# muellan/metacache

Hardware: AMD Instinct MI355X
Metric: Mreads/min (150 bp) (higher is better)
Workload: dtype u32

## Files before the change

### metacache_amd/csrc/gw_kernels.hip

```cpp
#include "device_common.h"

#include <algorithm>
#include <cstdlib>

namespace mcamd {

namespace {

constexpr uint32_t kGwNone = 0xFFFFFFFFu;
constexpr uint32_t kGwRounds = 128;
constexpr uint32_t kGwLoads = kGwRounds / 16;

struct __attribute__((packed, aligned(4))) U4 { uint32_t x, y, z, w; };

__device__ __forceinline__ uint32_t gw_block_shift(uint32_t maxWin)
{
    const uint32_t D = maxWin > 1 ? maxWin - 1 : 1;
    const uint32_t A = 32u - (uint32_t)__builtin_clz(64u * D - 1u);
    return A < 8u ? 8u : A;
}

template <uint32_t T1LOG2, uint32_t T2LOG2>
struct GwBloom {
    static constexpr uint32_t kW1 = (1u << T1LOG2) / 32, kW2 = (1u << T2LOG2) / 32, kWords = kW1 + kW2;
// ... 60 lines not shown
    }
    __device__ __forceinline__ static bool seen(const uint32_t* bits, uint32_t key)
    {
        const uint32_t h = hash(key), m = mask_of(h);
        return (bits[seen_index(h)] & m) == m;
    }
};

struct GwFrame {
    uint32_t A, D, blockMask, inner;
    uint32_t shv, Dsh, twoDsh;
    __device__ __forceinline__ explicit GwFrame(uint32_t maxWin, bool fine = false)
    {
        A = gw_block_shift(maxWin); D = maxWin > 1 ? maxWin - 1 : 0u;
        if (fine) { A = 32u - (uint32_t)__builtin_clz((D > 1u ? D : 2u) - 1u); A = A < 8u ? 8u : A; }
        blockMask = (1u << A) - 1u; inner = (1u << A) - 2u * D;
        const uint32_t sh = 32u - A;
        asm volatile("v_mov_b32 %0, %1" : "=v"(shv) : "s"(sh));
        Dsh = D << sh; twoDsh = (2u * D) << sh;
    }
    __device__ __forceinline__ bool edge(uint32_t v) const
    {
        uint32_t t;
        asm("v_lshl_add_u32 %0, %1, %2, %3" : "=v"(t) : "v"(v), "v"(shv), "s"(Dsh));
        return t < twoDsh;
    }
};

__device__ __forceinline__ void gw_fill_rounds(uint64_t* T, uint32_t lane, uint32_t r0, uint32_t Rc, uint32_t start, uint32_t myR, uint32_t sz, uint64_t pay)
{
    for (uint32_t i = lane; i < kGwRounds; i += 64) if (r0 + i >= Rc) T[i] = 0ull;
    const uint32_t jlo = r0 > start ? r0 - start : 0u, jhi = min(myR, r0 + kGwRounds > start ? r0 + kGwRounds - start : 0u);
    for (uint32_t j = jlo; j < jhi; ++j) T[start + j - r0] = (pay + 16ull * j) | ((uint64_t)min(16u, sz - 16u * j) << 40);
}
__device__ __forceinline__ uint32_t gw_lane_value(uint32_t v, int src) { return (uint32_t)__builtin_amdgcn_ds_bpermute(src << 2, (int)v); }
__device__ __forceinline__ void gw_fill_rounds_scan(uint64_t* T, uint32_t* E, uint32_t lane, uint32_t Rc, uint32_t start, uint32_t myR, uint32_t sz, uint64_t pay)
{
    E[lane] = 0u; E[lane + 64u] = 0u;
    wave_lds_sync();
    if (myR && start < kGwRounds) E[start] = lane + 1u;
    wave_lds_sync();
    uint32_t lo = wave_incl_scan_max_u32(E[lane]);
    uint32_t hi = max(wave_incl_scan_max_u32(E[lane + 64u]), rdlane(lo, 63));
    const uint32_t payLo = (uint32_t)pay, payHi = (uint32_t)(pay >> 32);
#pragma unroll
    for (uint32_t h = 0; h < 2; ++h) {
        const uint32_t slot = lane + 64u * h, who = h ? hi : lo;
        const int src = (int)(who ? who - 1u : 0u);
        const uint32_t eStart = gw_lane_value(start, src), eSz = gw_lane_value(sz, src);
        const uint32_t eLo = gw_lane_value(payLo, src), eHi = gw_lane_value(payHi, src);
        const uint32_t j = slot - eStart;
        const uint64_t ep = ((uint64_t)eHi << 32) | eLo;
        T[slot] = (who && slot < Rc) ? ((ep + 16ull * j) | ((uint64_t)min(16u, eSz - 16u * j) << 40)) : 0ull;
    }
}
__device__ __forceinline__ void gw_fill_rounds_scan_at(uint64_t* T, uint32_t* E, uint32_t lane, uint32_t r0, uint32_t Rc, uint32_t start, uint32_t myR, uint32_t sz, uint64_t pay)
{
    E[lane] = 0u; E[lane + 64u] = 0u;
    wave_lds_sync();
    if (myR && start < r0 + kGwRounds && start + myR > r0) E[start > r0 ? start - r0 : 0u] = lane + 1u;
    wave_lds_sync();
    uint32_t lo = wave_incl_scan_max_u32(E[lane]);
    uint32_t hi = max(wave_incl_scan_max_u32(E[lane + 64u]), rdlane(lo, 63));
    const uint32_t payLo = (uint32_t)pay, payHi = (uint32_t)(pay >> 32);
#pragma unroll
    for (uint32_t h = 0; h < 2; ++h) {
        const uint32_t slot = lane + 64u * h, who = h ? hi : lo;
        const int src = (int)(who ? who - 1u : 0u);
        const uint32_t eStart = gw_lane_value(start, src), eSz = gw_lane_value(sz, src);
        const uint32_t eLo = gw_lane_value(payLo, src), eHi = gw_lane_value(payHi, src);
        const uint32_t j = r0 + slot - eStart;
        const uint64_t ep = ((uint64_t)eHi << 32) | eLo;
        T[slot] = (who && r0 + slot < Rc) ? ((ep + 16ull * j) | ((uint64_t)min(16u, eSz - 16u * j) << 40)) : 0ull;
    }
}
__device__ __forceinline__ uint4 gw_left_as_is()
{
    uint4 r;
    asm volatile("" : "=v"(r.x), "=v"(r.y), "=v"(r.z), "=v"(r.w));
    return r;
}
template <bool BARE = false>
__device__ __forceinline__ void gw_load_rounds(const uint64_t* T, const uint32_t* __restrict__ values32, uint32_t grp, uint32_t sub4, uint4 (&x)[kGwLoads],
                                               uint32_t nl = kGwLoads)
{
#pragma unroll
    for (uint32_t u = 0; u < kGwLoads; ++u) {
        x[u] = make_uint4(kGwNone, kGwNone, kGwNone, kGwNone);
        if (u >= nl) continue;
        if constexpr (BARE) { x[u] = gw_left_as_is(); x[u].x = kGwNone; }
        const uint64_t rd = T[u * 16 + grp];
        if (sub4 < (uint32_t)(rd >> 40)) {
            const U4 t = *reinterpret_cast<const U4*>(values32 + (rd & 0xFFFFFFFFFFull) + sub4);
            x[u] = make_uint4(t.x, t.y, t.z, t.w);
        }
    }
}
template <class Bloom, bool LEAVE = false>
__device__ __forceinline__ void gw_mark_rounds(uint32_t* bits, const uint4 (&x)[kGwLoads], uint32_t A, uint32_t nl = kGwLoads)
{
#pragma unroll
    for (uint32_t u = 0; u < kGwLoads; ++u) {
        if (u >= nl) { if constexpr (LEAVE) break; else continue; }
        if (x[u].x != kGwNone) Bloom::mark4(bits, x[u].x >> A, x[u].y >> A, x[u].z >> A, x[u].w >> A);
    }
}
struct GwSink { uint32_t* dst; uint32_t room, n2; uint32_t* shared = nullptr; };
__device__ __forceinline__ uint32_t gw_reserve(uint32_t* shared, uint32_t tot)
{
    uint32_t at = 0;
    if (tot && __builtin_amdgcn_mbcnt_hi(~0u, __builtin_amdgcn_mbcnt_lo(~0u, 0u)) == 0u) at = atomicAdd(shared, tot);
    return (uint32_t)__builtin_amdgcn_readfirstlane((int)at);
}
template <class Bloom, bool FINE = false>
__device__ __forceinline__ void gw_take(const uint32_t* bits, const GwFrame& F, GwSink& S, uint32_t v, bool valid)
{
    const uint32_t key = v >> F.A;
    const bool keep = valid & (FINE ? (Bloom::twice(bits, key) | Bloom::seen(bits, key - 1u) | Bloom::seen(bits, key + 1u)) : (Bloom::twice(bits, key) | F.edge(v)));
    const uint64_t m = __ballot(keep);
    if (S.shared) S.n2 = gw_reserve(S.shared, (uint32_t)__popcll(m));
    if (keep) {
        const uint32_t at = __builtin_amdgcn_mbcnt_hi((uint32_t)(m >> 32), __builtin_amdgcn_mbcnt_lo((uint32_t)m, S.n2));
        if (at < S.room) S.dst[at] = v;
    }
    S.n2 += (uint32_t)__popcll(m);
}
constexpr int kGwFits = 0, kGwLaneRoom = 1, kGwWaveRoom = 2;
template <class Bloom, int CHECK, bool FINE = false>
__device__ __forceinline__ void gw_take4(const uint32_t* bits, const GwFrame& F, GwSink& S, const uint4 x, const int32_t rem)
{
    const uint32_t v[4] = {x.x, x.y, x.z, x.w};
    uint32_t m[4], wd[4];
    uint32_t mlo[FINE ? 4 : 1], wlo[FINE ? 4 : 1], mhi[FINE ? 4 : 1], whi[FINE ? 4 : 1];
#pragma unroll
    for (int j = 0; j < 4; ++j) {
        const uint32_t key = v[j] >> F.A;
        const uint32_t h = Bloom::hash(key);
        m[j] = h;
        wd[j] = bits[Bloom::twice_index(Bloom::seen_index(h), h)];
        if constexpr (FINE) {
            const uint32_t h0 = Bloom::hash(key - 1u), h1 = Bloom::hash(key + 1u);
            mlo[j] = Bloom::mask_of(h0); wlo[j] = bits[Bloom::seen_index(h0)];
            mhi[j] = Bloom::mask_of(h1); whi[j] = bits[Bloom::seen_index(h1)];
        }
    }
    uint64_t km[4]; bool kb[4];
#pragma unroll
    for (int j = 0; j < 4; ++j) {
        const bool valid = rem > j, hit = Bloom::twice_hit_h(wd[j], m[j]);
        if constexpr (FINE) {
            const bool lo = (wlo[j] & mlo[j]) == mlo[j], hi = (whi[j] & mhi[j]) == mhi[j];
            kb[j] = valid & (hit | lo | hi);
            km[j] = __ballot(valid) & (__ballot(hit) | __ballot(lo) | __ballot(hi));
        } else {
            const bool edge = F.edge(v[j]);
            kb[j] = valid & (hit | edge);
            km[j] = __ballot(valid) & (__ballot(hit) | __ballot(edge));
        }
    }
    if (S.shared) S.n2 = gw_reserve(S.shared, (uint32_t)(__popcll(km[0]) + __popcll(km[1]) + __popcll(km[2]) + __popcll(km[3])));
    uint32_t n2 = S.n2;
    if constexpr (CHECK == kGwWaveRoom) {
        const uint32_t end = n2 + (uint32_t)__popcll(km[0]) + (uint32_t)__popcll(km[1]) + (uint32_t)__popcll(km[2]) + (uint32_t)__popcll(km[3]);
        if (end <= S.room) {
#pragma unroll
            for (int j = 0; j < 4; ++j) {
                if (kb[j]) {
                    const uint32_t mine = __builtin_amdgcn_mbcnt_hi((uint32_t)(km[j] >> 32), __builtin_amdgcn_mbcnt_lo((uint32_t)km[j], 0u));
                    (S.dst + n2)[mine] = v[j];
                }
                n2 += (uint32_t)__popcll(km[j]);
            }
        }
        S.n2 = end;
        return;
    }
#pragma unroll
    for (int j = 0; j < 4; ++j) {
        if (kb[j]) {
// ... 471 lines not shown
        const uint32_t mv = wave_min_u32(hh == mh ? hv : kGwNone);
        const uint32_t winner = __ffsll((unsigned long long)__ballot(hh == mh && hv == mv)) - 1;
        const uint32_t d = rdlane(hd, winner);
        if constexpr (TAX) {
            const uint32_t g = rdlane(hg, winner);
#pragma unroll
            for (uint32_t r = 0; r < PER; ++r) if (ptax[r] == g) live &= ~(1u << r);
        } else {
            const uint32_t from = mv - tab.gwGap, span = 2u * tab.gwGap;
#pragma unroll
            for (uint32_t r = 0; r < PER; ++r) if (v[r] - from <= span) live &= ~(1u << r);
        }
        if (lane == rnd) { wv = mv; wh = mh; wd = d; }
        strong += mh >= 2 ? 1u : 0u;
    }
    owv = wv; owh = wh; owd = wd;
    return strong;
}

template <bool TAX>
__device__ __forceinline__ bool gw_winners_out(const uint32_t lane, const uint32_t K, const uint32_t wv, const uint32_t wh, const uint32_t wd,
                                               const uint32_t wt, const uint32_t wlo, const uint32_t whi, mc_candidate_dev* __restrict__ out,
                                               uint32_t (&pickLo)[kLaneK], uint32_t (&pickHi)[kLaneK])
{
    bool again = false;
    if constexpr (!TAX) {
#pragma unroll
        for (uint32_t i = 0; i + 1 < kLaneK; ++i) {
            const uint32_t ti = rdlane(wt, i);
            again = again || (__ballot(lane > i && lane < K && wt == ti && ti != 0xFFFFFFFFu) != 0);
        }
    }
#pragma unroll
    for (uint32_t i = 0; i < kLaneK; ++i) { pickLo[i] = rdlane(wlo, i); pickHi[i] = rdlane(whi, i); }
    if (lane < K) {
        mc_candidate_dev e; e.tgt = wt; e.hits = wh; e.end = wv - wlo; e.beg = e.end - wd;
        if (wv == kGwNone) { e.tgt = 0xFFFFFFFFu; e.hits = 0; e.beg = 0; e.end = 0; }
        out[lane] = e;
    }
    return again;
}

}

namespace {

__device__ __forceinline__ void lk_store_entries(const Workspace& ws, const uint32_t fbase, const uint32_t nf, const uint32_t lane, const uint32_t sz, const uint64_t pay,
                                                 const uint64_t fm, const uint64_t sm, const uint32_t lincl)
{
    const uint32_t nent = (uint32_t)__popcll(fm), n1 = (uint32_t)__popcll(sm), lsz = sz > 1u ? sz : 0u;
    const uint32_t below = __builtin_amdgcn_mbcnt_hi((uint32_t)(fm >> 32), __builtin_amdgcn_mbcnt_lo((uint32_t)fm, 0u));
    const uint32_t sbelow = __builtin_amdgcn_mbcnt_hi((uint32_t)(sm >> 32), __builtin_amdgcn_mbcnt_lo((uint32_t)sm, 0u));
    if (sz != 0u) {
        const uint32_t slot = sz == 1u ? sbelow : n1 + (below - sbelow);
        const uint32_t off = sz == 1u ? slot : n1 + lincl - lsz;
        ws.psize[fbase + slot] = sz | ((off & kEntOffMask) << 16);
        ws.ppay[fbase + slot] = pay;
    } else if (lane < nf) ws.psize[fbase + nent + (lane - below)] = 0u;
}
__device__ __forceinline__ void lk_store_entries(const Workspace& ws, const uint32_t fbase, const uint32_t nf, const uint32_t lane, const uint32_t sz, const uint64_t pay)
{
    lk_store_entries(ws, fbase, nf, lane, sz, pay, __ballot(sz != 0u), __ballot(sz == 1u), wave_incl_scan_u32(sz > 1u ? sz : 0u, lane));
}
__device__ __forceinline__ void lk_load_entries(const Workspace& ws, const DeviceTable& tab, const uint32_t s, const uint32_t q, const uint32_t lane,
                                                uint32_t& fbase, uint32_t& nf, uint32_t& sz, uint64_t& pay)
{
    const uint32_t o0 = ws.winOff[q];
    fbase = o0 * s; nf = (ws.winOff[q + 1] - o0) * s;
    const uint32_t f = lane < nf ? ws.features[fbase + lane] : 0xFFFFFFFFu;
    const uint64_t e = f != 0xFFFFFFFFu ? tab.direct[f] : 0ull;
    sz = (uint32_t)e & 0xFFFFu; pay = direct_payload(e);
}

struct GwEntRecord {
    const uint4* rec;
    __device__ __forceinline__ uint2 where() const { const uint4 r6 = *rec; return make_uint2(r6.y, rec_entries(r6.z)); }
    __device__ __forceinline__ void load(const Workspace& ws, const DeviceTable&, uint32_t, uint32_t fbase, uint32_t nent, uint32_t lane, uint32_t& sz, uint64_t& pay) const
    {
        sz = lane < nent ? (ws.psize[fbase + lane] & 0xFFFFu) : 0u;
        pay = lane < nent ? ws.ppay[fbase + lane] : 0ull;
    }
    __device__ __forceinline__ void leave(const Workspace&, const DeviceTable&, uint32_t, uint32_t) const {}
};
struct GwEntLookup {
    uint32_t fbase, nent, s;
    __device__ __forceinline__ uint2 where() const { return make_uint2(fbase, nent); }
    __device__ __forceinline__ void load(const Workspace& ws, const DeviceTable& tab, uint32_t q, uint32_t, uint32_t, uint32_t lane, uint32_t& sz, uint64_t& pay) const
    {
        uint32_t fb, nf;
        lk_load_entries(ws, tab, s, q, lane, fb, nf, sz, pay);
    }
    __device__ __forceinline__ void leave(const Workspace& ws, const DeviceTable& tab, uint32_t q, uint32_t lane) const
    {
        uint32_t fb, nf, sz; uint64_t pay;
        lk_load_entries(ws, tab, s, q, lane, fb, nf, sz, pay);
        lk_store_entries(ws, fb, nf, lane, sz, pay);
    }
};

struct GwPend {
    bool pend = false;
    uint32_t q = 0, wv = kGwNone, whd = 0, dir = 0, b0 = 0, b1 = 0, b2 = 0;
    __device__ __forceinline__ void bases(const DeviceTable& tab)
    {
        b0 = b1 = b2 = 0u;
        if (pend && wv != kGwNone) { b0 = tab.gwBase[dir]; b1 = tab.gwBase[dir + 1]; b2 = tab.gwBase[min(dir + 2, tab.gwTargets)]; }
    }
    template <bool TAX, class Ent>
    __device__ __forceinline__ void finish(const uint32_t lane, const uint32_t K, const DeviceTable& tab, const Workspace& ws, mc_candidate_dev* __restrict__ cands, const Ent& ent)
    {
        if (!pend) return;
        uint32_t t = 0xFFFFFFFFu, lo = 0, hi = 0;
        if (wv != kGwNone) {
            t = dir; lo = b0; hi = b1;
            if (wv >= b1) { ++t; lo = b1; hi = b2; }
            while (wv >= hi) { ++t; lo = hi; hi = tab.gwBase[t + 1]; }
        }
        uint32_t plo[kLaneK], phi[kLaneK];
        const bool again = gw_winners_out<TAX>(lane, K, wv, whd & 0xFFFFu, whd >> 16, t, lo, hi, cands + (size_t)q * K, plo, phi);
        if (again) ent.leave(ws, tab, q, lane);
        if (lane == 0) {
            if (again) { ws.hitScan[q] = ws.qstat[q].hits; ws.qflag[q] = kFlagCands; }
            else ws.qflag[q] = kFlagDone;
        }
        pend = false;
    }
};

template <uint32_t LOG2S, bool TAX, bool DEFER, bool LONG = false, class GetV, class Ent>
__device__ __forceinline__ bool gw_count_read(const uint32_t q, const Ent& ent, const uint32_t n2, const uint32_t maxWin, GetV&& getv,
                                              uint2* slots, uint32_t* ck, uint64_t* T, const uint32_t lane, const uint32_t grp, const uint32_t sub4,
                                              const uint32_t K, const uint32_t* __restrict__ taxkey, const DeviceTable& tab, const Workspace& ws,
                                              mc_candidate_dev* __restrict__ cands, GwPend& P)
{
    constexpr uint32_t kSlots = 1u << LOG2S, kList = kSlots / 2;
    {
        uint4* k4 = reinterpret_cast<uint4*>(slots);
#pragma unroll
        for (uint32_t i = 0; i < kSlots * 8 / 16 / 64; ++i) k4[i * 64 + lane] = make_uint4(kGwNone, 0u, kGwNone, 0u);
    }
    wave_lds_sync();
    uint32_t pickLo[kLaneK], pickHi[kLaneK];
#pragma unroll
    for (uint32_t i = 0; i < kLaneK; ++i) { pickLo[i] = 0; pickHi[i] = 0; }
    uint32_t strong = 0, wv = kGwNone, wh = 0, wd = 0;
    bool again = false;
    mc_candidate_dev* out = cands + (size_t)q * K;
    if constexpr (DEFER) P.bases(tab);
    uint32_t C = 0;
    auto body = [&](auto perc) {
        constexpr uint32_t PER = decltype(perc)::value;
        uint32_t v[PER];
#pragma unroll
        for (uint32_t r = 0; r < PER; ++r) v[r] = getv(r);
        C = gw_count_numbers<LOG2S, PER, LONG ? kList : 0xFFFFFFFFu>(v, slots, ck, lane);
    };
    const uint32_t per = (n2 + 63u) / 64u;
    if constexpr (LOG2S == 9) {
        if (per <= 1) body(std::integral_constant<uint32_t, 1>{});
        else if (per <= 2) body(std::integral_constant<uint32_t, 2>{});
        else if (per <= 3) body(std::integral_constant<uint32_t, 3>{});
        else if (!LONG || per <= 4) body(std::integral_constant<uint32_t, 4>{});
        else if constexpr (LONG) {
            if (per <= 6) body(std::integral_constant<uint32_t, 6>{});
            else body(std::integral_constant<uint32_t, 8>{});
        }
    } else if constexpr (LOG2S == 10) {
        if (per <= 6) body(std::integral_constant<uint32_t, 6>{});
        else body(std::integral_constant<uint32_t, 8>{});
    } else {
        if (per <= 10) body(std::integral_constant<uint32_t, 10>{});
        else if (per <= 12) body(std::integral_constant<uint32_t, 12>{});
        else body(std::integral_constant<uint32_t, kList / 64>{});
    }
    C = __builtin_amdgcn_readfirstlane(C);
    wave_lds_sync();
    if constexpr (LONG) {
        if (C > kList) {
            if constexpr (DEFER) P.template finish<TAX>(lane, K, tab, ws, cands, ent);
// ... 106 lines not shown
                ent.leave(ws, tab, q, lane);
                if (lane == 0) { ws.hitScan[q] = ws.qstat[q].hits; ws.qflag[q] = kFlagCands; }
                done = false;
            }
        }
    }
    if (done && lane == 0) ws.qflag[q] = kFlagDone;
    wave_lds_sync();
    return true;
}

}

#ifndef MC_GW_COUNT_WPE
#define MC_GW_COUNT_WPE 6
#endif
template <uint32_t LOG2S, uint32_t WAVES, bool TAX>
__global__ __launch_bounds__(WAVES * 64, LOG2S == 9 ? MC_GW_COUNT_WPE : LOG2S == 10 ? 5 : 1) void gw_count_kernel(BatchView b, uint32_t s, DeviceTable tab, Workspace ws, uint32_t K,
                                                                                             const uint32_t* __restrict__ taxkey, mc_candidate_dev* __restrict__ cands,
                                                                                             uint32_t minN2)
{
    constexpr uint32_t kSlots = 1u << LOG2S, kList = kSlots / 2;
    static_assert(kGwRounds * 8 <= kSlots * 8, "step D's round table lives in the slot table, which is done with by then");
    __shared__ __attribute__((aligned(16))) uint2 slotS[WAVES][kSlots];
    __shared__ uint32_t ckS[WAVES][kList];
    const uint32_t lane = threadIdx.x & 63u, wave = __builtin_amdgcn_readfirstlane(threadIdx.x >> 6);
    uint2* slots = slotS[wave];
    uint32_t* ck = ckS[wave];
    uint64_t* T = reinterpret_cast<uint64_t*>(slotS[wave]);
    const uint32_t total = ws.midCount[kCntFilter];
    const uint4* __restrict__ work = ws.midList + list_at(kListFiltered, b.n);
    const uint4* __restrict__ work6 = ws.midList + list_at(kListFilter, b.n);
    const uint32_t nWaves = gridDim.x * WAVES;
    const uint32_t w0 = blockIdx.x * WAVES + wave;
    const uint32_t grp = lane >> 2, sub4 = (lane & 3u) * 4u;
    const uint32_t* __restrict__ pool = reinterpret_cast<const uint32_t*>(ws.bigPool);
    constexpr uint32_t kPre = LOG2S <= 10 ? kList / 64 : 1;
    uint32_t pre[kPre];
    auto fetch = [&](uint32_t off, uint32_t n) {
        if constexpr (LOG2S <= 10) {
#pragma unroll
            for (uint32_t r = 0; r < kPre; ++r) pre[r] = r * 64 + lane < n ? pool[off + r * 64 + lane] : kGwNone;
        }
    };
    constexpr bool kDefer = LOG2S <= 10;
    GwPend P;
    const uint32_t nmine = LOG2S == 9 ? total : ws.midCount[LOG2S == 10 ? kCnt512 : kCnt1024];
    const uint32_t kStep = LOG2S == 9 ? 64u : min(8u, max(1u, (nmine + nWaves - 1) / nWaves));
    const uint32_t* __restrict__ side = ws.sideList + list_at(LOG2S == 10 ? kSide512 : kSide1024, b.n);
    for (uint32_t chunk = w0 * kStep; chunk < nmine; chunk += nWaves * kStep) {
      const bool inb = lane < kStep && chunk + lane < nmine;
      const uint32_t myW = LOG2S == 9 ? chunk + lane : (inb ? side[chunk + lane] : 0u);
      const uint4 myRec = inb ? work[myW] : make_uint4(0, 0, kGwFallback, 0);
      uint64_t todo = __ballot(myRec.z <= kList && (minN2 == 0 || myRec.z > minN2) && myRec.w <= kHashWin);
      if (todo) { const uint32_t j = (uint32_t)__ffsll((unsigned long long)todo) - 1; fetch(rdlane(myRec.y, j), rdlane(myRec.z, j)); }
      while (todo) {
        const uint32_t j = (uint32_t)__ffsll((unsigned long long)todo) - 1;
        todo &= todo - 1;
        const uint32_t w = rdlane(myW, j), q = rdlane(myRec.x, j), n2 = rdlane(myRec.z, j), maxWin = rdlane(myRec.w, j);
        const uint32_t* __restrict__ src = pool + rdlane(myRec.y, j);
        uint32_t cur[kPre];
#pragma unroll
        for (uint32_t r = 0; r < kPre; ++r) cur[r] = pre[r];
        if (todo) { const uint32_t jn = (uint32_t)__ffsll((unsigned long long)todo) - 1; fetch(rdlane(myRec.y, jn), rdlane(myRec.z, jn)); }
        gw_count_read<LOG2S, TAX, kDefer>(q, GwEntRecord{work6 + w}, n2, maxWin, [&](uint32_t r) -> uint32_t {
            if constexpr (LOG2S <= 10) return cur[r < kPre ? r : 0];
            else return r * 64 + lane < n2 ? src[r * 64 + lane] : kGwNone;
        }, slots, ck, T, lane, grp, sub4, K, taxkey, tab, ws, cands, P);
      }
    }
    if constexpr (kDefer) { P.bases(tab); P.template finish<TAX>(lane, K, tab, ws, cands, GwEntRecord{work6}); }
}

constexpr uint32_t kGwCounted = 0x80000000u;

template <uint32_t WAVES, uint32_t TLOG2, bool TAX, uint32_t WPE = MC_GW_FILTER_WPE, bool LOOKUP = false>
__global__ __launch_bounds__(WAVES * 64, WPE) void gw_filter_count_kernel(BatchView b, DeviceTable tab, Workspace ws, uint32_t K, const uint32_t* __restrict__ taxkey,
                                                                                 mc_candidate_dev* __restrict__ cands, const uint32_t s)
{
    using Bloom = GwBloom<TLOG2, TLOG2>;
    constexpr uint32_t kKeep = WPE >= 6 ? 384 : 512;
    static_assert(kGwRounds * 8 >= 256 * 4, "the distinct numbers' slots take the place of the round table");
    constexpr bool kSeven = WPE >= 7;
    __shared__ __attribute__((aligned(16))) uint32_t bitS[WAVES][Bloom::kWords];
    __shared__ __attribute__((aligned(16))) uint64_t roundS[kSeven ? 1 : WAVES][kSeven ? 1 : kGwRounds];
    __shared__ __attribute__((aligned(16))) uint32_t keptS[WAVES][kKeep];
    uint32_t lane = threadIdx.x & 63u;
    const uint32_t wave = __builtin_amdgcn_readfirstlane(threadIdx.x >> 6);
    uint32_t* bits = bitS[wave];
    uint64_t* T = kSeven ? reinterpret_cast<uint64_t*>(bits) : roundS[kSeven ? 0 : wave];
    uint32_t* kept = keptS[wave];
    const uint32_t total = LOOKUP ? b.n : ws.midCount[kCntFilter];
    uint4* const work = ws.midList + list_at(kListFilter, b.n);
    uint4* __restrict__ outRec = ws.midList + list_at(kListFiltered, b.n);
    const uint32_t nWaves = gridDim.x * WAVES;
    const uint32_t w0 = blockIdx.x * WAVES + wave;
    auto load_rec = [&](uint32_t w) -> uint4 { return (!LOOKUP && w < total) ? work[w] : make_uint4(0, 0, 0, 0); };
    const uint64_t sliceCap = ws.bigPoolCap / nWaves;
    uint32_t* const slice = reinterpret_cast<uint32_t*>(ws.bigPool) + (uint64_t)w0 * sliceCap;
    uint64_t sliceUsed = (LOOKUP && ws.sliceFill) ? ws.sliceFill[w0] : 0u;
    uint32_t deferred = 0;
    uint4 rec = load_rec(w0), recNext = load_rec(w0 + nWaves);
    uint32_t esz = 0; uint64_t epay = 0;
    auto load_entries = [&](const uint4& r) {
        if constexpr (LOOKUP) return;
        const uint32_t ne = rec_hits(r.z) <= kGwSmallH ? min(rec_entries(r.z), 64u) : 0u;
        esz = lane < ne ? ws.psize[r.y + lane] : 0u;
        epay = lane < ne ? ws.ppay[r.y + lane] : 0ull;
    };
    load_entries(rec);
    constexpr uint32_t kLkSkip = 0xFFFFFFFFu;
    auto load_raw = [&](uint32_t q) -> uint32_t {
        uint32_t raw = 0u;
        if (LOOKUP && q < b.n && lane < 3u) raw = *(lane < 2u ? ws.winOff + q + lane : ws.qflag + q);
        return raw;
    };
    auto decode_raw = [&](uint32_t raw) -> uint2 {
        const uint32_t o0 = rdlane(raw, 0), nf = (rdlane(raw, 1) - o0) * s;
        return (LOOKUP && rdlane(raw, 2) == kFlagProbe && nf <= 64u) ? make_uint2(o0 * s, nf) : make_uint2(kLkSkip, 0u);
    };
    auto load_feat = [&](const uint2& m) -> uint32_t { return (m.x != kLkSkip && lane < m.y) ? ws.features[m.x + lane] : 0xFFFFFFFFu; };
    uint2 mA = make_uint2(kLkSkip, 0u), mB = mA;
    uint32_t lkFeat = 0xFFFFFFFFu, lkNfeat = 0, lkRaw = 0; uint64_t lkEnt = 0;
    if constexpr (LOOKUP) {
        mA = decode_raw(load_raw(w0)); mB = decode_raw(load_raw(w0 + nWaves));
        const uint32_t f0 = load_feat(mA);
        lkFeat = load_feat(mB);
        lkRaw = load_raw(w0 + 2 * nWaves);
        lkNfeat = (uint32_t)__popcll(__ballot(f0 != 0xFFFFFFFFu));
        lkEnt = f0 != 0xFFFFFFFFu ? tab.direct[f0] : 0ull;
    }
    uint32_t grp = lane >> 2, sub4 = (lane & 3u) * 4u;
    auto hide_lane = [&]() {
        if constexpr (LOOKUP) { asm volatile("" : "+v"(lane)); grp = lane >> 2; sub4 = (lane & 3u) * 4u; }
    };
    GwPend P;
    for (uint32_t w = w0; w < total; w += nWaves) {
      bool advanced = false;
      auto advance = [&]() {
          if constexpr (LOOKUP) { lkFeat = load_feat(mB); lkRaw = load_raw(w + 3 * nWaves); advanced = true; }
      };
      do {
        uint32_t q, nent, H, maxWin, sz, fbase = 0, nfs = 0; uint64_t pay;
        uint32_t rix = 0xFFFFFFFFu;
        if constexpr (!LOOKUP) {
            q = rec.x; nent = rec_entries(rec.z); H = rec_hits(rec.z); maxWin = rec.w;
            sz = esz & 0xFFFFu; pay = epay;
            rec = recNext;
            recNext = load_rec(w + 2 * nWaves);
            load_entries(rec);
        } else {
            hide_lane();
            const uint2 cur = mA; const uint64_t e = lkEnt; const uint32_t nfeat = lkNfeat;
            const uint2 mC = decode_raw(lkRaw);
            lkNfeat = (uint32_t)__popcll(__ballot(lkFeat != 0xFFFFFFFFu));
            lkEnt = lkFeat != 0xFFFFFFFFu ? tab.direct[lkFeat] : 0ull;
            mA = mB; mB = mC;
            if (cur.x == kLkSkip) continue;
            q = w; fbase = cur.x; nfs = cur.y;
            sz = (uint32_t)e & 0xFFFFu; pay = direct_payload(e);
            const uint64_t fm = __ballot(sz != 0u), sm = __ballot(sz == 1u);
            nent = (uint32_t)__popcll(fm);
            const uint32_t n1 = (uint32_t)__popcll(sm), lsz = sz > 1u ? sz : 0u;
            const uint32_t lincl = wave_incl_scan_u32(lsz, lane);
            H = n1 + rdlane(lincl, 63);
            maxWin = b.max_win(q);
            if (lane == 0) { QueryStat qs; qs.hits = H; qs.nfeat = nfeat; qs.nfound = nent; qs.nsteps = nfeat; ws.qstat[q] = qs; }
            if (H == 0) {
                if (lane < K) { mc_candidate_dev ev; ev.tgt = 0xFFFFFFFFu; ev.hits = 0; ev.beg = 0; ev.end = 0; cands[(size_t)q * K + lane] = ev; }
                if (lane == 0) { ws.hitScan[q] = 0u; ws.qflag[q] = kFlagDone; }
                continue;
            }
            const uint32_t cls = read_class(H, nent, maxWin, ClassLimits{ws.bigMin, tab.gwGap, true});
            if (lane == 0) {
                ws.hitScan[q] = segment_hits(H, cls);
                ws.qflag[q] = cls != kClassWave ? kFlagMid : kFlagCands;
                if (cls != kClassWave && cls != kClassFilter) {
                    const uint32_t at = atomicAdd(&ws.midCount[class_counter(cls)], 1u);
                    ws.midList[list_at(class_list(cls), b.n) + at] = as_uint4(work_record(q, fbase, nent, H, maxWin));
                }
            }
            if (cls != kClassFilter) { lk_store_entries(ws, fbase, nfs, lane, sz, pay, fm, sm, lincl); continue; }
        }
        auto entries_out = [&]() { if constexpr (LOOKUP) GwEntLookup{fbase, nent, s}.leave(ws, tab, q, lane); };
        auto slot_of = [&]() -> uint32_t {
            if constexpr (!LOOKUP) return w;
            else {
                if (rix == 0xFFFFFFFFu) {
                    uint32_t at = 0;
                    if (lane == 0) { at = atomicAdd(&ws.midCount[kCntFilter], 1u); work[at] = as_uint4(work_record(q, fbase, nent, H, maxWin)); }
                    rix = rdlane(at, 0);
                }
                return rix;
            }
        };
        const uint32_t myR = sz > 1 ? (sz + 15u) >> 4 : 0u;
        const uint32_t incl = wave_incl_scan_u32(myR, lane), Rc = rdlane(incl, 63);
        if (H > kGwSmallH || nent > 64u || Rc > kGwRounds || maxWin > tab.gwGap || sliceCap - sliceUsed < kGwRounds * 16u + 64u) {
            if constexpr (LOOKUP) lk_store_entries(ws, fbase, nfs, lane, sz, pay);
            const uint32_t at = slot_of();
            if (lane == 0) outRec[at] = make_uint4(q, 0u, kGwDefer, maxWin);
            ++deferred;
            continue;
        }
        auto clear_bits = [&]() {
            uint4* z4 = reinterpret_cast<uint4*>(bits);
#pragma unroll
            for (uint32_t i = 0; i < Bloom::kWords / 4 / 64; ++i) z4[i * 64 + lane] = make_uint4(0, 0, 0, 0);
        };
        if constexpr (!kSeven) clear_bits();
        gw_fill_rounds_scan(T, kept, lane, Rc, incl - myR, myR, sz, pay);
        wave_lds_sync();
        const GwFrame F(maxWin);
        const uint32_t nl = (Rc + 15u) >> 4;
        const uint32_t svLow = sz == 1 ? (uint32_t)pay : 0u;
        const uint32_t svBase = sz == 1 ? tab.gwBase[(uint32_t)(pay >> 32)] : kGwNone;
        uint4 x[kGwLoads];
        gw_load_rounds<LOOKUP>(T, tab.values32, grp, sub4, x, nl);
        uint32_t svTop = svBase;
        uint32_t rems = 0;
        if constexpr (kSeven) {
            rems = gw_pack_rems<LOOKUP>(T, grp, sub4, nl);
            hide_lane();
            wave_lds_sync();
            clear_bits();
            wave_lds_sync();
            if constexpr (LOOKUP) asm volatile("" : "+v"(svTop));
        }
        const uint32_t sv = svTop + svLow;
        auto take_rounds = [&](auto check, GwSink& S) {
            constexpr int CHECK = decltype(check)::value;
            if constexpr (kSeven) gw_take_rounds_packed<Bloom, CHECK, LOOKUP>(bits, rems, F, S, x, nl);
            else gw_take_rounds<Bloom, CHECK>(bits, T, F, S, grp, sub4, x, nl);
        };
        if (sv != kGwNone) Bloom::mark(bits, sv >> F.A);
        gw_mark_rounds<Bloom, LOOKUP>(bits, x, F.A, nl);
        hide_lane();
        wave_lds_sync();
        const bool here = maxWin <= kHashWin;
        uint32_t n2;
        if (here) {
            GwSink S{kept, kKeep, 0u};
            gw_take<Bloom>(bits, F, S, sv, sv != kGwNone);
            take_rounds(std::integral_constant<int, LOOKUP ? kGwWaveRoom : kGwLaneRoom>{}, S);
            n2 = S.n2;
        } else {
            GwSink S{slice + sliceUsed, (uint32_t)min((uint64_t)kGwMaxKept, sliceCap - sliceUsed), 0u};
            gw_take<Bloom>(bits, F, S, sv, sv != kGwNone);
            take_rounds(std::integral_constant<int, kGwFits>{}, S);
            n2 = S.n2;
        }
        if (here && n2 <= kKeep) {
            hide_lane();
            advance();
            if constexpr (!LOOKUP) { if (lane == 0) outRec[w] = make_uint4(q, 0u, kGwCounted | n2, maxWin); }
            wave_lds_sync();
            auto count = [&](const auto& ent) {
                return gw_count_read<9, TAX, true, true>(q, ent, n2, maxWin,
                                        [&](uint32_t r) -> uint32_t { return r * 64 + lane < n2 ? kept[r * 64 + lane] : kGwNone; },
                                        reinterpret_cast<uint2*>(bits), kSeven ? kept : reinterpret_cast<uint32_t*>(T), kSeven ? reinterpret_cast<uint64_t*>(kept) : T,
                                        lane, grp, sub4, K, taxkey, tab, ws, cands, P);
            };
            bool counted;
            if constexpr (LOOKUP) counted = count(GwEntLookup{fbase, nent, s});
            else counted = count(GwEntRecord{work + w});
            if (!counted && kSeven) {
                entries_out();
                const uint32_t at = slot_of();
                if (lane == 0) outRec[at] = make_uint4(q, 0u, kGwDefer, maxWin);
                ++deferred;
                wave_lds_sync();
            } else if (!counted) {
#pragma unroll
                for (uint32_t r = 0; r < kKeep / 64; ++r) if (r * 64 + lane < n2) slice[sliceUsed + r * 64 + lane] = kept[r * 64 + lane];
                entries_out();
                const uint32_t at = slot_of();
                if (lane == 0) outRec[at] = make_uint4(q, (uint32_t)((uint64_t)w0 * sliceCap + sliceUsed), n2, maxWin);
                sliceUsed += n2;
                wave_lds_sync();
            }
            continue;
        }
        if (here) {
            GwSink S{slice + sliceUsed, (uint32_t)min((uint64_t)kGwMaxKept, sliceCap - sliceUsed), 0u};
            gw_take<Bloom>(bits, F, S, sv, sv != kGwNone);
            take_rounds(std::integral_constant<int, kGwFits>{}, S);
            n2 = S.n2;
        }
        const uint32_t room = (uint32_t)min((uint64_t)kGwMaxKept, sliceCap - sliceUsed);
        const bool fallback = n2 > room;
        entries_out();
        const uint32_t at = slot_of();
        if (lane == 0) {
            if (fallback) { ws.hitScan[q] = H; ws.qflag[q] = kFlagCands; outRec[at] = make_uint4(q, 0u, kGwFallback, maxWin); }
            else outRec[at] = make_uint4(q, (uint32_t)((uint64_t)w0 * sliceCap + sliceUsed), n2, maxWin);
        }
        if (!fallback) sliceUsed += n2;
        wave_lds_sync();
      } while (false);
      if (!advanced) advance();
    }
    P.bases(tab);
    if constexpr (LOOKUP) P.template finish<TAX>(lane, K, tab, ws, cands, GwEntLookup{0u, 0u, s});
    else P.template finish<TAX>(lane, K, tab, ws, cands, GwEntRecord{work});
    if (lane == 0) {
        if (ws.sliceFill) ws.sliceFill[w0] = (uint32_t)sliceUsed;
        if (deferred) atomicAdd(&ws.midCount[kCntSecond], deferred);
    }
}

constexpr uint32_t kGwBigSorted = 8192;

template <bool TAX>
__device__ __forceinline__ void gw_sorted_scan(const uint32_t* __restrict__ g, const uint32_t first, const uint32_t end, const uint32_t D,
                                               const DeviceTable& tab, const uint32_t* __restrict__ taxkey, const uint32_t K, uint32_t* ring,
                                               const uint32_t lane, LaneCand (&top)[kLaneK], uint32_t (&toptax)[kLaneK])
{
    uint32_t cT = 0xFFFFFFFFu, cHits = 0, cBeg = 0, cEnd = 0, cLo = 0, cHi = 0;
    uint32_t lowFst = 0;
    uint32_t gnext = first + lane < end ? g[first + lane] : 0xFFFFFFFFu;
    uint32_t dnext = gnext != 0xFFFFFFFFu ? tab.gwDir[gnext >> tab.gwDirShift] : 0u;
    for (uint32_t base = first; base < end; base += 64) {
        const uint32_t cnt = min(64u, end - base), ei = base + lane;
        const bool valid = lane < cnt;
        const uint32_t gi = gnext, di = dnext;
        gnext = ei + 64u < end ? g[ei + 64u] : 0xFFFFFFFFu;
        ring[ei & 127u] = gi;
        wave_lds_sync();
        const uint32_t want = gi - D;
        const uint32_t rlo = base >= first + 64u ? base - 64u : first;
        uint32_t lo = 0, hi = 0;
        bool glob = false;
        if (valid) {
            if (lowFst >= rlo) { lo = lowFst; hi = ei; }
            else if (ring[rlo & 127u] < want) { lo = rlo + 1u; hi = ei; }
            else { lo = lowFst; hi = rlo; glob = true; }
        }
        while (__ballot(!glob && lo < hi)) {
            const uint32_t mid = (lo + hi) >> 1;
            if (!glob && lo < hi) { if (ring[mid & 127u] < want) lo = mid + 1u; else hi = mid; }
        }
        while (__ballot(glob && lo < hi)) {
            const uint32_t mid = (lo + hi) >> 1;
            if (glob && lo < hi) { if (g[mid] < want) lo = mid + 1u; else hi = mid; }
        }
        const uint32_t fst = lo;
        const uint32_t gf = !valid ? 0u : fst >= rlo ? ring[fst & 127u] : g[fst];
        lowFst = rdlane(fst, cnt - 1u);
        uint32_t t = 0xFFFFFFFFu, tlo = 0, thi = 0;
        const bool inCur = cT != 0xFFFFFFFFu && (gi - cLo) < (cHi - cLo);
        if (valid) {
            if (inCur) { t = cT; tlo = cLo; thi = cHi; }
            else {
                t = di;
                const uint32_t b0 = tab.gwBase[t], b1 = tab.gwBase[t + 1], b2 = tab.gwBase[min(t + 2, tab.gwTargets)];
                tlo = b0; thi = b1;
                if (gi >= b1) { ++t; tlo = b1; thi = b2; }
                while (gi >= thi) { ++t; tlo = thi; thi = tab.gwBase[t + 1]; }
            }
        }
        if (cT != 0xFFFFFFFFu && rdlane(t, 0) != cT && lane == 0) {
            LaneCand c; c.tgt = cT; c.hits = cHits; c.beg = cBeg; c.end = cEnd;
            top_insert(top, toptax, c, K, TAX ? taxkey : nullptr, 0xFFFFFFFFu);
        }
        uint32_t val = valid ? (((ei - fst + 1u) << 6) | (63u - lane)) : 0u;
#pragma unroll
        for (uint32_t d = 1; d < 64; d <<= 1) {
            const uint32_t ov = (uint32_t)__shfl_up((int)val, d), ot = (uint32_t)__shfl_up((int)t, d);
            if (lane >= d && ot == t) val = max(val, ov);
        }
        const uint32_t tnext = (uint32_t)__shfl_down((int)t, 1);
        const bool tail = valid && (lane + 1u >= cnt || tnext != t);
        const uint32_t wl = 63u - (val & 63u);
        LaneCand c; c.tgt = t; c.hits = val >> 6;
        c.beg = (uint32_t)__shfl((int)gf, (int)wl) - tlo; c.end = (uint32_t)__shfl((int)gi, (int)wl) - tlo;
        if (t == cT && cHits >= c.hits) { c.hits = cHits; c.beg = cBeg; c.end = cEnd; }
        const bool last = base + 64u >= end;
        if (tail && (last || lane + 1u < cnt)) top_insert(top, toptax, c, K, TAX ? taxkey : nullptr, 0xFFFFFFFFu);
        cT = rdlane(c.tgt, cnt - 1u); cHits = rdlane(c.hits, cnt - 1u); cBeg = rdlane(c.beg, cnt - 1u); cEnd = rdlane(c.end, cnt - 1u);
        cLo = rdlane(tlo, cnt - 1u); cHi = rdlane(thi, cnt - 1u);
        dnext = gnext != 0xFFFFFFFFu ? tab.gwDir[gnext >> tab.gwDirShift] : 0u;
    }
    wave_lds_sync();
}

template <bool TAX, class Put>
__device__ __forceinline__ uint32_t gw_sorted_rounds(LaneCand (&top)[kLaneK], uint32_t (&toptax)[kLaneK], const uint32_t K, Put&& put)
{
    uint32_t strong = 0;
    for (uint32_t rnd = 0; rnd < K; ++rnd) {
// ... 176 lines not shown
```

Baseline: 23550.

## Reload cold workspace pointers from kernarg to cut live SGPRs in fused lookup kernel

In the LOOKUP instance of the filter-count kernel, rarely used workspace pointers (psize, ppay, midCount, midList, sliceFill, bigPool) are re-read from the kernarg segment at each point of use instead of being held in registers for the whole kernel. Opaque asm barriers keep the compiler from hoisting those reloads. The Bloom bits and kept buffers are also merged into one per-wave LDS struct, and the remainder packing is computed inside the bare round loader instead of in a separate pass over T. The aim is lower scalar and vector register pressure and fewer LDS reads, in exchange for extra scalar loads on cold paths.

```diff
diff --git a/metacache_amd/csrc/gw_kernels.hip b/metacache_amd/csrc/gw_kernels.hip
--- a/metacache_amd/csrc/gw_kernels.hip
+++ b/metacache_amd/csrc/gw_kernels.hip
@@ -166,8 +166,10 @@
 }
 template <bool BARE = false>
 __device__ __forceinline__ void gw_load_rounds(const uint64_t* T, const uint32_t* __restrict__ values32, uint32_t grp, uint32_t sub4, uint4 (&x)[kGwLoads],
-                                               uint32_t nl = kGwLoads)
-{
+                                               uint32_t nl = kGwLoads,
+                                               uint32_t* rems = nullptr)
+{
+    uint32_t packed = 0;
 #pragma unroll
     for (uint32_t u = 0; u < kGwLoads; ++u) {
         x[u] = make_uint4(kGwNone, kGwNone, kGwNone, kGwNone);
@@ -177,8 +179,10 @@
         if (sub4 < (uint32_t)(rd >> 40)) {
             const U4 t = *reinterpret_cast<const U4*>(values32 + (rd & 0xFFFFFFFFFFull) + sub4);
             x[u] = make_uint4(t.x, t.y, t.z, t.w);
-        }
-    }
+            if constexpr (BARE) packed |= min((uint32_t)(rd >> 40) - sub4, 4u) << (3u * u);
+        }
+    }
+    if constexpr (BARE) *rems = packed;
 }
 template <class Bloom, bool LEAVE = false>
 __device__ __forceinline__ void gw_mark_rounds(uint32_t* bits, const uint4 (&x)[kGwLoads], uint32_t A, uint32_t nl = kGwLoads)
@@ -816,6 +820,20 @@
     }
     __device__ __forceinline__ void leave(const Workspace&, const DeviceTable&, uint32_t, uint32_t) const {}
 };
+struct GwFusedArgs { BatchView b; DeviceTable tab; Workspace ws; uint32_t K; const uint32_t* taxkey; mc_candidate_dev* cands; uint32_t s; };
+__device__ __forceinline__ Workspace gw_cold_ws()
+{
+    using KernArg = const __attribute__((address_space(4))) char*;
+    KernArg p = (KernArg)__builtin_amdgcn_kernarg_segment_ptr();
+    asm volatile("" : "+s"(p));
+    Workspace w;
+#define MC_GW_COLD(f) w.f = *reinterpret_cast<const __attribute__((address_space(4))) decltype(Workspace::f)*>(p + offsetof(GwFusedArgs, ws) + offsetof(Workspace, f))
+    MC_GW_COLD(psize); MC_GW_COLD(ppay); MC_GW_COLD(midCount); MC_GW_COLD(midList); MC_GW_COLD(sliceFill); MC_GW_COLD(bigPool);
+#undef MC_GW_COLD
+    return w;
+}
+__device__ __forceinline__ uint32_t gw_opaque(uint32_t v) { asm volatile("" : "+s"(v)); return v; }
+
 struct GwEntLookup {
     uint32_t fbase, nent, s;
     __device__ __forceinline__ uint2 where() const { return make_uint2(fbase, nent); }
@@ -828,7 +846,7 @@
     {
         uint32_t fb, nf, sz; uint64_t pay;
         lk_load_entries(ws, tab, s, q, lane, fb, nf, sz, pay);
-        lk_store_entries(ws, fb, nf, lane, sz, pay);
+        lk_store_entries(gw_cold_ws(), fb, nf, lane, sz, pay);
     }
 };
 
@@ -1101,6 +1119,9 @@
     constexpr uint32_t kKeep = WPE >= 6 ? 384 : 512;
     static_assert(kGwRounds * 8 >= 256 * 4, "the distinct numbers' slots take the place of the round table");
     constexpr bool kSeven = WPE >= 7;
+    if constexpr (LOOKUP) {
+        asm volatile("" : "+s"(tab.gwGap), "+s"(tab.gwDirShift));
+    }
     __shared__ __attribute__((aligned(16))) uint32_t bitS[WAVES][Bloom::kWords];
     __shared__ __attribute__((aligned(16))) uint64_t roundS[kSeven ? 1 : WAVES][kSeven ? 1 : kGwRounds];
     __shared__ __attribute__((aligned(16))) uint32_t keptS[WAVES][kKeep];
@@ -1109,15 +1130,24 @@
     uint32_t* bits = bitS[wave];
     uint64_t* T = kSeven ? reinterpret_cast<uint64_t*>(bits) : roundS[kSeven ? 0 : wave];
     uint32_t* kept = keptS[wave];
+    struct __attribute__((aligned(16))) WaveLds { uint32_t bits[Bloom::kWords]; uint32_t kept[kKeep]; };
+    __shared__ WaveLds waveS[LOOKUP ? WAVES : 1];
+    if constexpr (LOOKUP) { static_assert(kSeven, "LOOKUP is a seven-wave instance"); bits = waveS[wave].bits; kept = waveS[wave].kept; T = reinterpret_cast<uint64_t*>(bits); }
+    auto cold = [&]() -> std::conditional_t<LOOKUP, Workspace, const Workspace&> { if constexpr (LOOKUP) return gw_cold_ws(); else return ws; };
     const uint32_t total = LOOKUP ? b.n : ws.midCount[kCntFilter];
-    uint4* const work = ws.midList + list_at(kListFilter, b.n);
-    uint4* __restrict__ outRec = ws.midList + list_at(kListFiltered, b.n);
+    uint4* const work = LOOKUP ? nullptr : ws.midList + list_at(kListFilter, b.n);
+    uint4* __restrict__ outRec = LOOKUP ? nullptr : ws.midList + list_at(kListFiltered, b.n);
+    auto work_of = [&](const Workspace& c) -> uint4* { if constexpr (LOOKUP) return c.midList + list_at(kListFilter, gw_opaque(total)); else return work; };
+    auto out_of = [&](const Workspace& c) -> uint4* { if constexpr (LOOKUP) return c.midList + list_at(kListFiltered, gw_opaque(total)); else return outRec; };
     const uint32_t nWaves = gridDim.x * WAVES;
     const uint32_t w0 = blockIdx.x * WAVES + wave;
     auto load_rec = [&](uint32_t w) -> uint4 { return (!LOOKUP && w < total) ? work[w] : make_uint4(0, 0, 0, 0); };
     const uint64_t sliceCap = ws.bigPoolCap / nWaves;
-    uint32_t* const slice = reinterpret_cast<uint32_t*>(ws.bigPool) + (uint64_t)w0 * sliceCap;
-    uint64_t sliceUsed = (LOOKUP && ws.sliceFill) ? ws.sliceFill[w0] : 0u;
+    uint32_t* const slice = LOOKUP ? nullptr : reinterpret_cast<uint32_t*>(ws.bigPool) + (uint64_t)w0 * sliceCap;
+    auto slice_at = [&]() -> uint64_t { if constexpr (LOOKUP) return (uint64_t)gw_opaque(w0) * sliceCap; else return (uint64_t)w0 * sliceCap; };
+    auto slice_of = [&](const Workspace& c) -> uint32_t* { if constexpr (LOOKUP) return reinterpret_cast<uint32_t*>(c.bigPool) + slice_at(); else return slice; };
+    uint64_t sliceUsed = 0u;
+    if constexpr (LOOKUP) { const Workspace c = cold(); if (c.sliceFill) sliceUsed = c.sliceFill[w0]; }
     uint32_t deferred = 0;
     uint4 rec = load_rec(w0), recNext = load_rec(w0 + nWaves);
     uint32_t esz = 0; uint64_t epay = 0;
@@ -1195,11 +1225,12 @@
                 ws.hitScan[q] = segment_hits(H, cls);
                 ws.qflag[q] = cls != kClassWave ? kFlagMid : kFlagCands;
                 if (cls != kClassWave && cls != kClassFilter) {
-                    const uint32_t at = atomicAdd(&ws.midCount[class_counter(cls)], 1u);
-                    ws.midList[list_at(class_list(cls), b.n) + at] = as_uint4(work_record(q, fbase, nent, H, maxWin));
+                    const Workspace c = cold();
+                    const uint32_t at = atomicAdd(&c.midCount[class_counter(cls)], 1u);
+                    c.midList[list_at(class_list(cls), b.n) + at] = as_uint4(work_record(q, fbase, nent, H, maxWin));
                 }
             }
-            if (cls != kClassFilter) { lk_store_entries(ws, fbase, nfs, lane, sz, pay, fm, sm, lincl); continue; }
+            if (cls != kClassFilter) { lk_store_entries(cold(), fbase, nfs, lane, sz, pay, fm, sm, lincl); continue; }
         }
         auto entries_out = [&]() { if constexpr (LOOKUP) GwEntLookup{fbase, nent, s}.leave(ws, tab, q, lane); };
         auto slot_of = [&]() -> uint32_t {
@@ -1207,7 +1238,7 @@
             else {
                 if (rix == 0xFFFFFFFFu) {
                     uint32_t at = 0;
-                    if (lane == 0) { at = atomicAdd(&ws.midCount[kCntFilter], 1u); work[at] = as_uint4(work_record(q, fbase, nent, H, maxWin)); }
+                    if (lane == 0) { const Workspace c = cold(); at = atomicAdd(&c.midCount[kCntFilter], 1u); work_of(c)[at] = as_uint4(work_record(q, fbase, nent, H, maxWin)); }
                     rix = rdlane(at, 0);
                 }
                 return rix;
@@ -1216,9 +1247,9 @@
         const uint32_t myR = sz > 1 ? (sz + 15u) >> 4 : 0u;
         const uint32_t incl = wave_incl_scan_u32(myR, lane), Rc = rdlane(incl, 63);
         if (H > kGwSmallH || nent > 64u || Rc > kGwRounds || maxWin > tab.gwGap || sliceCap - sliceUsed < kGwRounds * 16u + 64u) {
-            if constexpr (LOOKUP) lk_store_entries(ws, fbase, nfs, lane, sz, pay);
+            if constexpr (LOOKUP) lk_store_entries(cold(), fbase, nfs, lane, sz, pay);
             const uint32_t at = slot_of();
-            if (lane == 0) outRec[at] = make_uint4(q, 0u, kGwDefer, maxWin);
+            if (lane == 0) out_of(cold())[at] = make_uint4(q, 0u, kGwDefer, maxWin);
             ++deferred;
             continue;
         }
@@ -1235,11 +1266,11 @@
         const uint32_t svLow = sz == 1 ? (uint32_t)pay : 0u;
         const uint32_t svBase = sz == 1 ? tab.gwBase[(uint32_t)(pay >> 32)] : kGwNone;
         uint4 x[kGwLoads];
-        gw_load_rounds<LOOKUP>(T, tab.values32, grp, sub4, x, nl);
+        uint32_t rems = 0;
+        gw_load_rounds<LOOKUP>(T, tab.values32, grp, sub4, x, nl, &rems);
         uint32_t svTop = svBase;
-        uint32_t rems = 0;
         if constexpr (kSeven) {
-            rems = gw_pack_rems<LOOKUP>(T, grp, sub4, nl);
+            if constexpr (!LOOKUP) rems = gw_pack_rems<false>(T, grp, sub4, nl);
             hide_lane();
             wave_lds_sync();
             clear_bits();
@@ -1264,7 +1295,7 @@
             take_rounds(std::integral_constant<int, LOOKUP ? kGwWaveRoom : kGwLaneRoom>{}, S);
             n2 = S.n2;
         } else {
-            GwSink S{slice + sliceUsed, (uint32_t)min((uint64_t)kGwMaxKept, sliceCap - sliceUsed), 0u};
+            GwSink S{slice_of(cold()) + sliceUsed, (uint32_t)min((uint64_t)kGwMaxKept, sliceCap - sliceUsed), 0u};
             gw_take<Bloom>(bits, F, S, sv, sv != kGwNone);
             take_rounds(std::integral_constant<int, kGwFits>{}, S);
             n2 = S.n2;
@@ -1286,22 +1317,23 @@
             if (!counted && kSeven) {
                 entries_out();
                 const uint32_t at = slot_of();
-                if (lane == 0) outRec[at] = make_uint4(q, 0u, kGwDefer, maxWin);
+                if (lane == 0) out_of(cold())[at] = make_uint4(q, 0u, kGwDefer, maxWin);
                 ++deferred;
                 wave_lds_sync();
             } else if (!counted) {
-#pragma unroll
-                for (uint32_t r = 0; r < kKeep / 64; ++r) if (r * 64 + lane < n2) slice[sliceUsed + r * 64 + lane] = kept[r * 64 + lane];
+                uint32_t* const to = slice_of(cold());
+#pragma unroll
+                for (uint32_t r = 0; r < kKeep / 64; ++r) if (r * 64 + lane < n2) to[sliceUsed + r * 64 + lane] = kept[r * 64 + lane];
                 entries_out();
                 const uint32_t at = slot_of();
-                if (lane == 0) outRec[at] = make_uint4(q, (uint32_t)((uint64_t)w0 * sliceCap + sliceUsed), n2, maxWin);
+                if (lane == 0) out_of(cold())[at] = make_uint4(q, (uint32_t)(slice_at() + sliceUsed), n2, maxWin);
                 sliceUsed += n2;
                 wave_lds_sync();
             }
             continue;
         }
         if (here) {
-            GwSink S{slice + sliceUsed, (uint32_t)min((uint64_t)kGwMaxKept, sliceCap - sliceUsed), 0u};
+            GwSink S{slice_of(cold()) + sliceUsed, (uint32_t)min((uint64_t)kGwMaxKept, sliceCap - sliceUsed), 0u};
             gw_take<Bloom>(bits, F, S, sv, sv != kGwNone);
             take_rounds(std::integral_constant<int, kGwFits>{}, S);
             n2 = S.n2;
@@ -1311,8 +1343,9 @@
         entries_out();
         const uint32_t at = slot_of();
         if (lane == 0) {
-            if (fallback) { ws.hitScan[q] = H; ws.qflag[q] = kFlagCands; outRec[at] = make_uint4(q, 0u, kGwFallback, maxWin); }
-            else outRec[at] = make_uint4(q, (uint32_t)((uint64_t)w0 * sliceCap + sliceUsed), n2, maxWin);
+            uint4* const o = out_of(cold());
+            if (fallback) { ws.hitScan[q] = H; ws.qflag[q] = kFlagCands; o[at] = make_uint4(q, 0u, kGwFallback, maxWin); }
+            else o[at] = make_uint4(q, (uint32_t)(slice_at() + sliceUsed), n2, maxWin);
         }
         if (!fallback) sliceUsed += n2;
         wave_lds_sync();
@@ -1323,8 +1356,9 @@
     if constexpr (LOOKUP) P.template finish<TAX>(lane, K, tab, ws, cands, GwEntLookup{0u, 0u, s});
     else P.template finish<TAX>(lane, K, tab, ws, cands, GwEntRecord{work});
     if (lane == 0) {
-        if (ws.sliceFill) ws.sliceFill[w0] = (uint32_t)sliceUsed;
-        if (deferred) atomicAdd(&ws.midCount[kCntSecond], deferred);
+        const auto& c = cold();
+        if (c.sliceFill) c.sliceFill[w0] = (uint32_t)sliceUsed;
+        if (deferred) atomicAdd(&c.midCount[kCntSecond], deferred);
     }
 }
 
```

New measurement: 23630, median of 6. About the same (+0.3%).
